# ishine/CatEars

Hardware: AMD Instinct MI355X
Metric: acoustic frames/sec (fbank->nnet posteriors), 16kHz, 1/2/4/8 GPU (higher is better)
Workload: dtype fp32 (bf16x6 GEMM: fp32 operands split exactly into 3 bf16 planes, 6 MFMA products, fp32 accumulate; every operand bit kept, dropped cross terms < 2^-25 |w x|; error vs oracle at the fp32-MFMA path's level, tests/test_gpu_parity.py)

## Files before the change

### catears_amd/csrc/kernels/gemm_bf16x6.hip

```cpp
#include <hip/hip_runtime.h>
#include <stdlib.h>

#include "../internal.h"
#include "../tile_order.h"

#ifndef CATEARS_X6_NT
#define CATEARS_X6_NT 0
#endif

namespace catears {
namespace {

typedef __bf16 bf16x8 __attribute__((ext_vector_type(8)));
typedef float f32x4 __attribute__((ext_vector_type(4)));
typedef float f32x2t __attribute__((ext_vector_type(2)));

struct X6Args {
  const uint16_t *w;
  const uint16_t *x;
  const float *wf, *xf;
  const float *bias, *bn_scale, *bn_offset;
  float *y32;
  uint16_t *y16;
  int ldw, pw, ldx, px, ldy, py;
// ... 420 lines not shown
          load_x(kt + 2, h);
          if (h == 1) read_plane(st, 2);
          __builtin_amdgcn_sched_barrier(0);
        }
#pragma unroll
        for (int i = 0; i < TW; ++i)
#pragma unroll
          for (int j = 0; j < TF; ++j) {
            acc[i][j] = __builtin_amdgcn_mfma_f32_16x16x32_bf16(a[0][i], b[2][j], acc[i][j], 0, 0, 0);
            acc[i][j] = __builtin_amdgcn_mfma_f32_16x16x32_bf16(a[2][i], b[0][j], acc[i][j], 0, 0, 0);
          }
        asm volatile("s_waitcnt lgkmcnt(0)" ::: "memory");
        __builtin_amdgcn_s_barrier();
      }
      asm volatile("s_waitcnt vmcnt(0)" ::: "memory");
      x6_epilogue<TW, TF, false>(p, acc, n0 + wrow, f0 + frow, lane);
      return;
    }
    for (int kt = 0; kt < ktiles; ++kt) {
      mfma_tile(kt);
      store(kt + 1);
      load(kt + 2);
      asm volatile("s_waitcnt lgkmcnt(0)" ::: "memory");
      if constexpr ((DIAG & 16) == 0) __builtin_amdgcn_s_barrier();
    }
    asm volatile("s_waitcnt vmcnt(0)" ::: "memory");
    x6_epilogue<TW, TF, false>(p, acc, n0 + wrow, f0 + frow, lane);
    return;
  }
  for (int kt = kbeg; kt < ktiles; ++kt) {
    store(kt + 1);
    load(kt + 2);
    const char *st = smem + (kt & 1) * STAGE;
    bf16x8 a[3][TW], b[3][TF];
#pragma unroll
    for (int pl = 0; pl < 3; ++pl) {
#pragma unroll
      for (int i = 0; i < TW; ++i)
        a[pl][i] = *reinterpret_cast<const bf16x8 *>(st + (pl * BW + wrow + i * 16) * 64 + foff);
#pragma unroll
      for (int j = 0; j < TF; ++j)
        b[pl][j] = *reinterpret_cast<const bf16x8 *>(st + 3 * BW * 64 + (pl * BF + frow + j * 16) * 64 + foff);
    }
#pragma unroll
    for (int i = 0; i < TW; ++i)
#pragma unroll
      for (int j = 0; j < TF; ++j) acc[i][j] = __builtin_amdgcn_mfma_f32_16x16x32_bf16(a[0][i], b[0][j], acc[i][j], 0, 0, 0);
#pragma unroll
    for (int i = 0; i < TW; ++i)
#pragma unroll
      for (int j = 0; j < TF; ++j) {
        acc[i][j] = __builtin_amdgcn_mfma_f32_16x16x32_bf16(a[0][i], b[1][j], acc[i][j], 0, 0, 0);
        acc[i][j] = __builtin_amdgcn_mfma_f32_16x16x32_bf16(a[1][i], b[0][j], acc[i][j], 0, 0, 0);
        acc[i][j] = __builtin_amdgcn_mfma_f32_16x16x32_bf16(a[1][i], b[1][j], acc[i][j], 0, 0, 0);
      }
#pragma unroll
    for (int i = 0; i < TW; ++i)
#pragma unroll
      for (int j = 0; j < TF; ++j) {
        acc[i][j] = __builtin_amdgcn_mfma_f32_16x16x32_bf16(a[0][i], b[2][j], acc[i][j], 0, 0, 0);
        acc[i][j] = __builtin_amdgcn_mfma_f32_16x16x32_bf16(a[2][i], b[0][j], acc[i][j], 0, 0, 0);
      }
    asm volatile("s_waitcnt lgkmcnt(0)" ::: "memory");
    __builtin_amdgcn_s_barrier();
  }
  asm volatile("s_waitcnt vmcnt(0)" ::: "memory");
  x6_epilogue<TW, TF, false>(p, acc, n0 + wrow, f0 + frow, lane);
}

template <class C, bool FIRST = false, int DIAG = 0, int KS = 1, bool PIN = false, bool OUT16 = false, int PRIO = 0>
__global__ __launch_bounds__(C::NT, 512 / C::NT) void gemm_bf16x6d_kernel(X6Args p) {
#ifndef CATEARS_DIAG
  static_assert(DIAG == 0, "ablation builds (wrong results) only with -DCATEARS_DIAG");
#endif
  static_assert(KS == 1 || (KS == 2 && !FIRST), "two K-tiles per stage: hidden layers only (even K-tile count)");
  static_assert(!PIN || (!FIRST && KS == 1 && DIAG == 0), "plane input: hidden / output layers, one K-tile per stage");
  constexpr int BF = C::BF, TW = C::TW, TF = C::TF, NT = C::NT;
  constexpr int RPP = NT / 4;
  static_assert(BF == RPP, "one activation row chunk per thread");
  constexpr int ASTAGE = 3 * BF * 64;
  __shared__ __attribute__((aligned(1024))) char smem[2 * KS * ASTAGE];
  auto stage_of = [&](int t) -> char * {
    if constexpr (KS == 1) return smem + (t & 1) * ASTAGE;
    else return smem + ((((t >> 1) & 1) << 1) + (t & 1)) * ASTAGE;
  };
  auto swz = [](int row) { return ((row >> 3) & 1) << 1; };
  typedef float f32x4v __attribute__((ext_vector_type(4)));
  typedef uint32_t u32x4 __attribute__((ext_vector_type(4)));
  typedef const __attribute__((address_space(1))) f32x4v gvec;
  typedef const __attribute__((address_space(1))) bf16x8 gfrag;
  typedef const __attribute__((address_space(1))) u32x4 gchunk;

  const int tid = threadIdx.x, lane = tid & 63, wave = tid >> 6;
  const int ww = wave / C::WGF, wf = wave % C::WGF;
  int tm, tn;
  tile_of(blockIdx.x, p.tiles_m, p.tiles_n, p.group, &tm, &tn);
  const int f0 = tm * BF, n0 = tn * C::BW;
  const int prow = tid >> 2, pch = tid & 3;
  const int ktiles = p.kpad / 32;

  gfrag *wb[TW];
#pragma unroll
  for (int i = 0; i < TW; ++i)
    wb[i] = (gfrag *)(p.wd + ((size_t)((n0 >> 4) + ww * TW + i) * p.wd_kt * 3 * 64 + lane) * 8);
  auto load_w = [&](int kt, int pl, bf16x8 *dst) {
    if constexpr ((DIAG & 8) != 0) {
      if (kt > 0) return;
    }
    kt = min(kt, ktiles - 1);
#pragma unroll
    for (int i = 0; i < TW; ++i) dst[i] = wb[i][(kt * 3 + pl) * 64];
  };
  f32x4v rx0[2], rx1[2];
  u32x4 rp[3][2];
  __shared__ int src_tab[FIRST ? 8 * BF : 1];
  if constexpr (FIRST) {
    for (int i = tid; i < 8 * BF; i += NT) {
      const int sg = i / BF, row = i % BF;
      const int shift = (int)(signed char)(p.off_packed >> (8 * min(sg, p.nseg - 1)));
      const int src = clampi(clampi(f0 + row, 0, p.m - 1) + shift, 0, p.m - 1);
      src_tab[i] = p.row_map ? p.row_map[src] : src;
    }
    __syncthreads();
  }
  auto load_x = [&](int kt, int r) {
    if constexpr ((DIAG & 4) != 0) {
      if (kt > 1) return;
    }
    kt = min(kt, ktiles - 1);
    const int k0 = kt * 32;
    if constexpr (FIRST) {
      const int k = k0 + 8 * pch, seg = k / p.din, segc = min(seg, p.nseg - 1);
      const int src = src_tab[segc * BF + prow];
      gvec *xb = (gvec *)(p.xf + (size_t)src * p.ldx + (seg < p.nseg ? k - segc * p.din : 0));
      rx0[r] = xb[0];
      rx1[r] = xb[1];
      if (seg >= p.nseg) rx0[r] = rx1[r] = f32x4v{0.0f, 0.0f, 0.0f, 0.0f};
    } else if constexpr (PIN) {
      const int seg = k0 / p.din, col0 = k0 - seg * p.din;
      const int shift = (int)(signed char)(p.off_packed >> (8 * seg));
      const int src = clampi(f0 + prow + shift, 0, p.m - 1);
      const uint32_t o = ((uint32_t)(src * p.ldx) + col0 + 8 * pch) / 8, ps = (uint32_t)p.px / 8;
      gchunk *xb = (gchunk *)p.x;
      rp[0][r] = xb[o];
      rp[1][r] = xb[o + ps];
      rp[2][r] = xb[o + 2 * ps];
    } else {
      const int seg = k0 / p.din, col0 = k0 - seg * p.din;
      const int shift = (int)(signed char)(p.off_packed >> (8 * seg));
      gvec *xb = (gvec *)(p.xf + col0 + 8 * pch);
      const int src = clampi(f0 + prow + shift, 0, p.m - 1);
      const uint32_t o = (uint32_t)(src * p.ldx) / 4;
      rx0[r] = xb[o];
      rx1[r] = xb[o + 1];
    }
  };
  auto put = [&](char *st, int r) {
    if constexpr ((DIAG & 2) != 0) return;
    if constexpr (PIN) {
      const int off = prow * 64 + ((pch ^ swz(prow)) * 16);
#pragma unroll
      for (int pl = 0; pl < 3; ++pl) *reinterpret_cast<u32x4 *>(st + pl * BF * 64 + off) = rp[pl][r];
      return;
    }
    Planes2 q0, q1, q2, q3;
    if constexpr ((DIAG & 1) != 0) {
      auto raw = [](float a, float b) {
        const uint32_t u = __builtin_bit_cast(uint32_t, a) ^ __builtin_bit_cast(uint32_t, b);
        return Planes2{u, u >> 1, u >> 2};
      };
      q0 = raw(rx0[r].x, rx0[r].y), q1 = raw(rx0[r].z, rx0[r].w);
      q2 = raw(rx1[r].x, rx1[r].y), q3 = raw(rx1[r].z, rx1[r].w);
    } else {
      q0 = split3_pair(rx0[r].x, rx0[r].y), q1 = split3_pair(rx0[r].z, rx0[r].w);
      q2 = split3_pair(rx1[r].x, rx1[r].y), q3 = split3_pair(rx1[r].z, rx1[r].w);
    }
    const int off = prow * 64 + ((pch ^ swz(prow)) * 16);
    *reinterpret_cast<u32x4 *>(st + off) = u32x4{q0.h, q1.h, q2.h, q3.h};
    *reinterpret_cast<u32x4 *>(st + BF * 64 + off) = u32x4{q0.m, q1.m, q2.m, q3.m};
    *reinterpret_cast<u32x4 *>(st + 2 * BF * 64 + off) = u32x4{q0.l, q1.l, q2.l, q3.l};
  };
  const int foff = (lane & 15) * 64 + (((lane >> 4) ^ (((lane >> 3) & 1) << 1)) * 16);
  const int frow = wf * TF * 16;
  auto read_b = [&](const char *st, int pl, bf16x8 *b) {
#pragma unroll
    for (int j = 0; j < TF; ++j) b[j] = *reinterpret_cast<const bf16x8 *>(st + (pl * BF + frow + j * 16) * 64 + foff);
  };

  f32x4 acc[TW][TF];
#pragma unroll
  for (int i = 0; i < TW; ++i)
#pragma unroll
    for (int j = 0; j < TF; ++j) acc[i][j] = f32x4{0.0f, 0.0f, 0.0f, 0.0f};

  bf16x8 a0[2][TW], a1[TW], a2[TW], b0[TF], b1[TF], b2[TF];
  load_x(0, 0);
  load_w(0, 0, a0[0]);
  load_w(0, 1, a1);
  load_w(0, 2, a2);
  if constexpr (KS == 1) {
    put(smem, 0);
    load_x(1, 1);
  } else {
    load_x(1, 1);
    put(stage_of(0), 0);
    put(stage_of(1), 1);
    load_x(2, 0);
  }
  asm volatile("s_waitcnt lgkmcnt(0)" ::: "memory");
  __builtin_amdgcn_s_barrier();

  auto body = [&](int kt, auto cc) {
    constexpr int c = decltype(cc)::value;
    const char *st = stage_of(kt);
    char *sn = stage_of(kt + KS);
    if constexpr (PRIO == 4) __builtin_amdgcn_s_setprio(1);
    read_b(st, 0, b0);
    read_b(st, 1, b1);
    if constexpr (PRIO == 4) __builtin_amdgcn_s_setprio(0);
    if constexpr (PRIO == 1 || PRIO == 3 || PRIO == 4 || PRIO == 5) __builtin_amdgcn_s_setprio(1);
    load_w(kt + 1, 0, a0[c ^ 1]);
    if constexpr (PRIO == 5) load_x(kt + KS + 1, KS == 1 ? c : c ^ 1);
    if constexpr (PRIO == 1 || PRIO == 3 || PRIO == 4 || PRIO == 5) __builtin_amdgcn_s_setprio(0);
    __builtin_amdgcn_sched_barrier(0);
    if constexpr (PRIO == 2) __builtin_amdgcn_s_setprio(1);
    if constexpr ((DIAG & 32) == 0) {
#pragma unroll
      for (int i = 0; i < TW; ++i)
#pragma unroll
        for (int j = 0; j < TF; ++j) acc[i][j] = __builtin_amdgcn_mfma_f32_16x16x32_bf16(a0[c][i], b0[j], acc[i][j], 0, 0, 0);
    }
    if constexpr (PRIO == 2) __builtin_amdgcn_s_setprio(0);
    __builtin_amdgcn_sched_barrier(0);
    if constexpr (PRIO == 1 || PRIO == 3 || PRIO == 4 || PRIO == 5) __builtin_amdgcn_s_setprio(1);
    if constexpr (PRIO != 5) load_x(kt + KS + 1, KS == 1 ? c : c ^ 1);
    if constexpr (PRIO == 1 || PRIO == 3 || PRIO == 4 || PRIO == 5) __builtin_amdgcn_s_setprio(0);
    __builtin_amdgcn_sched_barrier(0);
    if constexpr (PRIO == 2) __builtin_amdgcn_s_setprio(1);
    if constexpr (PRIO == 3) __builtin_amdgcn_s_setprio(1);
    put(sn, KS == 1 ? c ^ 1 : c);
    if constexpr (PRIO == 3) __builtin_amdgcn_s_setprio(0);
    if constexpr ((DIAG & 32) == 0) {
#pragma unroll
      for (int i = 0; i < TW; ++i)
#pragma unroll
        for (int j = 0; j < TF; ++j) {
          acc[i][j] = __builtin_amdgcn_mfma_f32_16x16x32_bf16(a0[c][i], b1[j], acc[i][j], 0, 0, 0);
          acc[i][j] = __builtin_amdgcn_mfma_f32_16x16x32_bf16(a1[i], b0[j], acc[i][j], 0, 0, 0);
          acc[i][j] = __builtin_amdgcn_mfma_f32_16x16x32_bf16(a1[i], b1[j], acc[i][j], 0, 0, 0);
        }
    }
    if constexpr (PRIO == 2) __builtin_amdgcn_s_setprio(0);
    if constexpr (PRIO == 4) __builtin_amdgcn_s_setprio(1);
    read_b(st, 2, b2);
    if constexpr (PRIO == 4) __builtin_amdgcn_s_setprio(0);
    __builtin_amdgcn_sched_barrier(0);
    if constexpr (PRIO == 1 || PRIO == 3 || PRIO == 4 || PRIO == 5) __builtin_amdgcn_s_setprio(1);
    load_w(kt + 1, 1, a1);
    if constexpr (PRIO == 1 || PRIO == 3 || PRIO == 4 || PRIO == 5) __builtin_amdgcn_s_setprio(0);
    __builtin_amdgcn_sched_barrier(0);
    if constexpr (PRIO == 2) __builtin_amdgcn_s_setprio(1);
    if constexpr ((DIAG & 32) == 0) {
#pragma unroll
      for (int i = 0; i < TW; ++i)
#pragma unroll
        for (int j = 0; j < TF; ++j) {
          acc[i][j] = __builtin_amdgcn_mfma_f32_16x16x32_bf16(a0[c][i], b2[j], acc[i][j], 0, 0, 0);
          acc[i][j] = __builtin_amdgcn_mfma_f32_16x16x32_bf16(a2[i], b0[j], acc[i][j], 0, 0, 0);
        }
    } else {
#pragma unroll
      for (int j = 0; j < TF; ++j) acc[0][j][0] += (float)b0[j][0] + (float)b1[j][0] + (float)b2[j][0] +
                                                   (float)a0[c][0][0] + (float)a1[0][0] + (float)a2[0][0];
    }
    if constexpr (PRIO == 2) __builtin_amdgcn_s_setprio(0);
    __builtin_amdgcn_sched_barrier(0);
    if constexpr (PRIO == 1 || PRIO == 3 || PRIO == 4 || PRIO == 5) __builtin_amdgcn_s_setprio(1);
    load_w(kt + 1, 2, a2);
    if constexpr (PRIO == 1 || PRIO == 3 || PRIO == 4 || PRIO == 5) __builtin_amdgcn_s_setprio(0);
    if constexpr (KS == 1 || c == 1) {
      asm volatile("s_waitcnt lgkmcnt(0)" ::: "memory");
      if constexpr ((DIAG & 16) == 0) __builtin_amdgcn_s_barrier();
    }
    __builtin_amdgcn_sched_barrier(0);
  };
  int kt = 0;
  for (; kt + 1 < ktiles; kt += 2) {
    body(kt, std::integral_constant<int, 0>());
    body(kt + 1, std::integral_constant<int, 1>());
  }
  if (KS == 1 && kt < ktiles) body(kt, std::integral_constant<int, 0>());
  asm volatile("s_waitcnt vmcnt(0)" ::: "memory");
  x6_epilogue<TW, TF, OUT16>(p, acc, n0 + ww * TW * 16, f0 + frow, lane);
}

template <int BW_, int BF_, int WGW_, int WGF_>
struct W6Cfg {
  static constexpr int BW = BW_, BF = BF_, WGW = WGW_, WGF = WGF_;
  static constexpr int NW = WGW * WGF, NT = 64 * NW;
  static constexpr int TW = BW / WGW / 16, TF = BF / WGF / 16;
  static_assert(TW * WGW * 16 == BW && TF * WGF * 16 == BF, "bad one-wave-per-SIMD tile");
};

template <class C, bool SG = false, int RING = 4>
__global__ __launch_bounds__(C::NT, C::NW / 4) void gemm_bf16x6w_kernel(X6Args p) {
  constexpr int BF = C::BF, TW = C::TW, TF = C::TF, NT = C::NT;
  static_assert(C::NW == 4 || C::NW == 8, "one or two waves per SIMD");
  static_assert(TW % RING == 0, "a ring of unit-block weight buffers that divides the unit blocks");
  constexpr int RQ = BF / (NT / 4);
  static_assert(RQ >= 1 && RQ * (NT / 4) == BF, "whole activation rows per thread");
  constexpr int ASTAGE = 3 * BF * 64;
  __shared__ __attribute__((aligned(1024))) char smem[2 * ASTAGE];
  auto swz = [](int row) { return ((row >> 3) & 1) << 1; };
  typedef float f32x4v __attribute__((ext_vector_type(4)));
  typedef uint32_t u32x4 __attribute__((ext_vector_type(4)));
  typedef const __attribute__((address_space(1))) f32x4v gvec;
  typedef const __attribute__((address_space(1))) bf16x8 gfrag;

  const int tid = threadIdx.x, lane = tid & 63, wave = tid >> 6;
  const int ww = wave / C::WGF, wf = wave % C::WGF;
  int tm, tn;
  tile_of(blockIdx.x, p.tiles_m, p.tiles_n, p.group, &tm, &tn);
  const int f0 = tm * BF, n0 = tn * C::BW;
  const int prow = tid >> 2, pch = tid & 3;
  const int ktiles = p.kpad / 32;

  gfrag *wbase = (gfrag *)(p.wd + ((size_t)((n0 >> 4) + ww * TW) * p.wd_kt * 3 * 64 + lane) * 8);
  bf16x8 wa[RING][3];
  auto load_w = [&](int kt, int i, int buf) {
    kt = min(kt, ktiles - 1);
#pragma unroll
    for (int pl = 0; pl < 3; ++pl) wa[buf][pl] = wbase[((size_t)(i * p.wd_kt + kt) * 3 + pl) * 64];
  };
  f32x4v rx0[RQ], rx1[RQ];
  auto load_x = [&](int kt) {
    kt = min(kt, ktiles - 1);
    const int k0 = kt * 32;
    const int seg = k0 / p.din, col0 = k0 - seg * p.din;
    const int shift = (int)(signed char)(p.off_packed >> (8 * seg));
    gvec *xb = (gvec *)(p.xf + col0 + 8 * pch);
#pragma unroll
    for (int q = 0; q < RQ; ++q) {
      const int src = clampi(f0 + prow + q * (NT / 4) + shift, 0, p.m - 1);
      const uint32_t o = (uint32_t)(src * p.ldx) / 4;
      rx0[q] = xb[o];
      rx1[q] = xb[o + 1];
    }
  };
  auto put = [&](char *st) {
#pragma unroll
    for (int q = 0; q < RQ; ++q) {
      const Planes2 q0 = split3_pair(rx0[q].x, rx0[q].y), q1 = split3_pair(rx0[q].z, rx0[q].w);
      const Planes2 q2 = split3_pair(rx1[q].x, rx1[q].y), q3 = split3_pair(rx1[q].z, rx1[q].w);
      const int row = prow + q * (NT / 4);
      const int off = row * 64 + ((pch ^ swz(row)) * 16);
      *reinterpret_cast<u32x4 *>(st + off) = u32x4{q0.h, q1.h, q2.h, q3.h};
      *reinterpret_cast<u32x4 *>(st + BF * 64 + off) = u32x4{q0.m, q1.m, q2.m, q3.m};
      *reinterpret_cast<u32x4 *>(st + 2 * BF * 64 + off) = u32x4{q0.l, q1.l, q2.l, q3.l};
    }
  };
  const int foff = (lane & 15) * 64 + (((lane >> 4) ^ (((lane >> 3) & 1) << 1)) * 16);
  const int frow = wf * TF * 16;
  auto frag = [&](const char *st, int pl, int j) {
    return *reinterpret_cast<const bf16x8 *>(st + (pl * BF + frow + j * 16) * 64 + foff);
  };

  f32x4 acc[TW][TF];
#pragma unroll
  for (int i = 0; i < TW; ++i)
#pragma unroll
    for (int j = 0; j < TF; ++j) acc[i][j] = f32x4{0.0f, 0.0f, 0.0f, 0.0f};
  bf16x8 b0[TF], b1[TF], b2[TF];

  load_x(0);
#pragma unroll
  for (int i = 0; i < RING - 1; ++i) load_w(0, i, i);
  put(smem);
  load_x(1);
  asm volatile("s_waitcnt lgkmcnt(0)" ::: "memory");
  __builtin_amdgcn_s_barrier();
#pragma unroll
  for (int j = 0; j < TF; ++j) {
    b0[j] = frag(smem, 0, j);
    b1[j] = frag(smem, 1, j);
    b2[j] = frag(smem, 2, j);
  }

  for (int kt = 0; kt < ktiles; ++kt) {
    char *sn = smem + ((kt + 1) & 1) * ASTAGE;
#pragma unroll
    for (int i = 0; i < TW; ++i) {
      load_w(kt + (i + RING - 1) / TW, (i + RING - 1) % TW, (i + RING - 1) % RING);
      if (i == 0) {
        if constexpr (!SG) {
          put(sn);
          load_x(kt + 2);
        }
      }
      __builtin_amdgcn_sched_barrier(0);
      if constexpr (SG) {
        if (i == 0) {
          put(sn);
          load_x(kt + 2);
#pragma unroll
          for (int g = 0; g < 6 * TF; ++g) {
            __builtin_amdgcn_sched_group_barrier(0x008, 1, 0);
            __builtin_amdgcn_sched_group_barrier(0x002, 2, 0);
            if (g % 4 == 3) __builtin_amdgcn_sched_group_barrier(0x200, 1, 0);
          }
        }
      }
      constexpr int u = 0;
#pragma unroll
      for (int j = 0; j < TF; ++j) {
        acc[i][j] = __builtin_amdgcn_mfma_f32_16x16x32_bf16(wa[i % RING][u], b0[j], acc[i][j], 0, 0, 0);
        acc[i][j] = __builtin_amdgcn_mfma_f32_16x16x32_bf16(wa[i % RING][u], b1[j], acc[i][j], 0, 0, 0);
        acc[i][j] = __builtin_amdgcn_mfma_f32_16x16x32_bf16(wa[i % RING][u + 1], b0[j], acc[i][j], 0, 0, 0);
        acc[i][j] = __builtin_amdgcn_mfma_f32_16x16x32_bf16(wa[i % RING][u + 1], b1[j], acc[i][j], 0, 0, 0);
        acc[i][j] = __builtin_amdgcn_mfma_f32_16x16x32_bf16(wa[i % RING][u], b2[j], acc[i][j], 0, 0, 0);
        acc[i][j] = __builtin_amdgcn_mfma_f32_16x16x32_bf16(wa[i % RING][u + 2], b0[j], acc[i][j], 0, 0, 0);
        if (i == TW - 1) {
          b0[j] = frag(sn, 0, j);
          b1[j] = frag(sn, 1, j);
          b2[j] = frag(sn, 2, j);
        }
      }
      if constexpr (SG) {
        if (i == TW - 1) {
#pragma unroll
          for (int j = 0; j < TF; ++j) {
            __builtin_amdgcn_sched_group_barrier(0x008, 6, 0);
            __builtin_amdgcn_sched_group_barrier(0x100, 3, 0);
          }
        }
      }
      if (i == TW / 2 - 1) {
        asm volatile("s_waitcnt lgkmcnt(0)" ::: "memory");
        __builtin_amdgcn_s_barrier();
      }
      __builtin_amdgcn_sched_barrier(0);
    }
  }
  asm volatile("s_waitcnt vmcnt(0) lgkmcnt(0)" ::: "memory");
  x6_epilogue<TW, TF, false>(p, acc, n0 + ww * TW * 16, f0 + frow, lane);
}

#ifdef CATEARS_EXPERIMENTS
template <class C>
__global__ __launch_bounds__(C::NT, 1) void gemm_bf16x6r_kernel(X6Args p) {
  constexpr int TW = C::TW, TF = C::TF;
  typedef float f32x4v __attribute__((ext_vector_type(4)));
  typedef uint32_t u32x4 __attribute__((ext_vector_type(4)));
  typedef const __attribute__((address_space(1))) f32x4v gvec;
  typedef const __attribute__((address_space(1))) bf16x8 gfrag;
  const int lane = threadIdx.x & 63, wave = threadIdx.x >> 6;
  const int ww = wave / C::WGF, wf = wave % C::WGF;
  int tm, tn;
  tile_of(blockIdx.x, p.tiles_m, p.tiles_n, p.group, &tm, &tn);
  const int f0 = tm * C::BF + wf * TF * 16, n0 = tn * C::BW;
  const int ktiles = p.kpad / 32;
  gfrag *wb[TW];
#pragma unroll
  for (int i = 0; i < TW; ++i)
    wb[i] = (gfrag *)(p.wd + ((size_t)((n0 >> 4) + ww * TW + i) * p.wd_kt * 3 * 64 + lane) * 8);
  int xrow[TF];
#pragma unroll
  for (int j = 0; j < TF; ++j) xrow[j] = f0 + 16 * j + (lane & 15);
  bf16x8 a[2][3][TW];
  f32x4v x[2][TF][2];
  auto load = [&](int kt, int buf) {
    kt = min(kt, ktiles - 1);
#pragma unroll
    for (int pl = 0; pl < 3; ++pl)
#pragma unroll
      for (int i = 0; i < TW; ++i) a[buf][pl][i] = wb[i][(kt * 3 + pl) * 64];
    const int k0 = kt * 32;
    const int seg = k0 / p.din, col = k0 - seg * p.din + 8 * (lane >> 4);
    const int shift = (int)(signed char)(p.off_packed >> (8 * seg));
#pragma unroll
    for (int j = 0; j < TF; ++j) {
      const int src = clampi(xrow[j] + shift, 0, p.m - 1);
      gvec *xp = (gvec *)(p.xf + (size_t)src * p.ldx + col);
      x[buf][j][0] = xp[0];
      x[buf][j][1] = xp[1];
    }
  };
  f32x4 acc[TW][TF];
#pragma unroll
  for (int i = 0; i < TW; ++i)
#pragma unroll
    for (int j = 0; j < TF; ++j) acc[i][j] = f32x4{0.0f, 0.0f, 0.0f, 0.0f};
  auto compute = [&](int buf) {
#pragma unroll
    for (int j = 0; j < TF; ++j) {
      const f32x4v v0 = x[buf][j][0], v1 = x[buf][j][1];
      const Planes2 q0 = split3_pair(v0.x, v0.y), q1 = split3_pair(v0.z, v0.w);
      const Planes2 q2 = split3_pair(v1.x, v1.y), q3 = split3_pair(v1.z, v1.w);
      const bf16x8 b0 = __builtin_bit_cast(bf16x8, u32x4{q0.h, q1.h, q2.h, q3.h});
      const bf16x8 b1 = __builtin_bit_cast(bf16x8, u32x4{q0.m, q1.m, q2.m, q3.m});
      const bf16x8 b2 = __builtin_bit_cast(bf16x8, u32x4{q0.l, q1.l, q2.l, q3.l});
#pragma unroll
      for (int i = 0; i < TW; ++i) acc[i][j] = __builtin_amdgcn_mfma_f32_16x16x32_bf16(a[buf][0][i], b0, acc[i][j], 0, 0, 0);
#pragma unroll
      for (int i = 0; i < TW; ++i) acc[i][j] = __builtin_amdgcn_mfma_f32_16x16x32_bf16(a[buf][0][i], b1, acc[i][j], 0, 0, 0);
#pragma unroll
      for (int i = 0; i < TW; ++i) acc[i][j] = __builtin_amdgcn_mfma_f32_16x16x32_bf16(a[buf][1][i], b0, acc[i][j], 0, 0, 0);
#pragma unroll
      for (int i = 0; i < TW; ++i) acc[i][j] = __builtin_amdgcn_mfma_f32_16x16x32_bf16(a[buf][1][i], b1, acc[i][j], 0, 0, 0);
#pragma unroll
      for (int i = 0; i < TW; ++i) acc[i][j] = __builtin_amdgcn_mfma_f32_16x16x32_bf16(a[buf][0][i], b2, acc[i][j], 0, 0, 0);
#pragma unroll
      for (int i = 0; i < TW; ++i) acc[i][j] = __builtin_amdgcn_mfma_f32_16x16x32_bf16(a[buf][2][i], b0, acc[i][j], 0, 0, 0);
    }
  };
  load(0, 0);
  int kt = 0;
  for (; kt + 1 < ktiles; kt += 2) {
    load(kt + 1, 1);
    __builtin_amdgcn_sched_barrier(0);
    compute(0);
    __builtin_amdgcn_sched_barrier(0);
    load(kt + 2, 0);
    __builtin_amdgcn_sched_barrier(0);
    compute(1);
    __builtin_amdgcn_sched_barrier(0);
  }
  if (kt < ktiles) compute(0);
  asm volatile("s_waitcnt vmcnt(0)" ::: "memory");
  x6_epilogue<TW, TF, false>(p, acc, n0 + ww * TW * 16, f0, lane);
}

#endif

template <class C, int NPV>
__global__ __launch_bounds__(C::NT + 64 * NPV, 1) void gemm_bf16x6ws_kernel(X6Args p) {
  constexpr int BW = C::BW, BF = C::BF, TW = C::TW, TF = C::TF, NT = C::NT, STAGE = C::STAGE;
  constexpr int RPP = 16 * NPV;
  static_assert((BW + BF) % RPP == 0, "rows per pass");
  constexpr int NP = (BW + BF) / RPP;
  __shared__ __attribute__((aligned(1024))) char smem[2 * STAGE];
  auto swz = [](int row) { return ((row >> 3) & 1) << 1; };
  typedef float f32x4v __attribute__((ext_vector_type(4)));
  typedef uint32_t u32x4 __attribute__((ext_vector_type(4)));
  typedef const __attribute__((address_space(1))) f32x4v gvec;

  const int tid = threadIdx.x, lane = tid & 63;
  const int wave = __builtin_amdgcn_readfirstlane(tid >> 6);
  int tm, tn;
  tile_of(blockIdx.x, p.tiles_m, p.tiles_n, p.group, &tm, &tn);
  const int f0 = tm * BF, n0 = tn * BW;
  const int ktiles = p.kpad / 32;

  if (wave >= C::NW) {
    const int pt = tid - NT, prow = pt >> 2, pch = pt & 3;
    bool isw[NP];
    int trow[NP];
    uint32_t wsrc[NP];
    int dst[NP];
#pragma unroll
    for (int i = 0; i < NP; ++i) {
      const int r = i * RPP + prow;
      isw[i] = BW % RPP == 0 ? i < BW / RPP : r < BW;
      trow[i] = isw[i] ? r : r - BW;
      wsrc[i] = (uint32_t)(min(n0 + trow[i], p.n - 1) * p.ldw + 8 * pch);
      dst[i] = (isw[i] ? 0 : 3 * BW * 64) + trow[i] * 64 + ((pch ^ swz(trow[i])) * 16);
    }
    f32x4v r0[NP], r1[NP];
    auto load = [&](int kt) {
      kt = min(kt, ktiles - 1);
      const int k0 = kt * 32;
      const int seg = k0 / p.din, col0 = k0 - seg * p.din;
      const int shift = (int)(signed char)(p.off_packed >> (8 * seg));
#pragma unroll
      for (int i = 0; i < NP; ++i) {
        gvec *src;
        if (isw[i]) {
          src = (gvec *)(p.wf + k0 + wsrc[i]);
        } else {
          const int x = clampi(f0 + trow[i] + shift, 0, p.m - 1);
          src = (gvec *)(p.xf + (uint32_t)(x * p.ldx) + col0 + 8 * pch);
        }
        r0[i] = src[0];
        r1[i] = src[1];
      }
    };
    auto store = [&](int kt) {
      char *st = smem + (kt & 1) * STAGE;
#pragma unroll
      for (int i = 0; i < NP; ++i) {
        const f32x4v v0 = r0[i], v1 = r1[i];
        const Planes2 q0 = split3_pair(v0.x, v0.y), q1 = split3_pair(v0.z, v0.w);
        const Planes2 q2 = split3_pair(v1.x, v1.y), q3 = split3_pair(v1.z, v1.w);
        const int ps = (isw[i] ? BW : BF) * 64;
        char *d = st + dst[i];
        *reinterpret_cast<u32x4 *>(d) = u32x4{q0.h, q1.h, q2.h, q3.h};
        *reinterpret_cast<u32x4 *>(d + ps) = u32x4{q0.m, q1.m, q2.m, q3.m};
        *reinterpret_cast<u32x4 *>(d + 2 * ps) = u32x4{q0.l, q1.l, q2.l, q3.l};
      }
    };
    load(0);
    store(0);
    load(1);
    asm volatile("s_waitcnt lgkmcnt(0)" ::: "memory");
    __builtin_amdgcn_s_barrier();
    for (int kt = 0; kt < ktiles; ++kt) {
      store(kt + 1);
      load(kt + 2);
      asm volatile("s_waitcnt lgkmcnt(0)" ::: "memory");
      __builtin_amdgcn_s_barrier();
    }
    asm volatile("s_waitcnt vmcnt(0)" ::: "memory");
    return;
  }

  const int ww = wave / C::WGF, wf = wave % C::WGF;
  const int foff = (lane & 15) * 64 + (((lane >> 4) ^ (((lane >> 3) & 1) << 1)) * 16);
  const int wrow = ww * TW * 16, frow = wf * TF * 16;
  f32x4 acc[TW][TF];
#pragma unroll
  for (int i = 0; i < TW; ++i)
#pragma unroll
    for (int j = 0; j < TF; ++j) acc[i][j] = f32x4{0.0f, 0.0f, 0.0f, 0.0f};
  __builtin_amdgcn_s_barrier();
  for (int kt = 0; kt < ktiles; ++kt) {
    const char *st = smem + (kt & 1) * STAGE;
    bf16x8 a[3][TW], b[3][TF];
#pragma unroll
    for (int pl = 0; pl < 3; ++pl) {
#pragma unroll
      for (int i = 0; i < TW; ++i)
        a[pl][i] = *reinterpret_cast<const bf16x8 *>(st + (pl * BW + wrow + i * 16) * 64 + foff);
#pragma unroll
      for (int j = 0; j < TF; ++j)
        b[pl][j] = *reinterpret_cast<const bf16x8 *>(st + 3 * BW * 64 + (pl * BF + frow + j * 16) * 64 + foff);
    }
#pragma unroll
    for (int i = 0; i < TW; ++i)
#pragma unroll
      for (int j = 0; j < TF; ++j) acc[i][j] = __builtin_amdgcn_mfma_f32_16x16x32_bf16(a[0][i], b[0][j], acc[i][j], 0, 0, 0);
#pragma unroll
    for (int i = 0; i < TW; ++i)
#pragma unroll
      for (int j = 0; j < TF; ++j) {
        acc[i][j] = __builtin_amdgcn_mfma_f32_16x16x32_bf16(a[0][i], b[1][j], acc[i][j], 0, 0, 0);
        acc[i][j] = __builtin_amdgcn_mfma_f32_16x16x32_bf16(a[1][i], b[0][j], acc[i][j], 0, 0, 0);
        acc[i][j] = __builtin_amdgcn_mfma_f32_16x16x32_bf16(a[1][i], b[1][j], acc[i][j], 0, 0, 0);
      }
#pragma unroll
    for (int i = 0; i < TW; ++i)
#pragma unroll
      for (int j = 0; j < TF; ++j) {
        acc[i][j] = __builtin_amdgcn_mfma_f32_16x16x32_bf16(a[0][i], b[2][j], acc[i][j], 0, 0, 0);
        acc[i][j] = __builtin_amdgcn_mfma_f32_16x16x32_bf16(a[2][i], b[0][j], acc[i][j], 0, 0, 0);
      }
    asm volatile("s_waitcnt lgkmcnt(0)" ::: "memory");
    __builtin_amdgcn_s_barrier();
  }
  x6_epilogue<TW, TF, false>(p, acc, n0 + wrow, f0 + frow, lane);
}

struct SpliceIdx8 {
  int v[8];
};

__global__ __launch_bounds__(256) void splice_pad_split_kernel(const float *__restrict__ in, int ld_in, int rows,
                                                               int din, int nseg, SpliceIdx8 idx,
                                                               const int *__restrict__ row_map,
                                                               uint16_t *__restrict__ out, int po) {
  const int r = blockIdx.x * 4 + (threadIdx.x >> 6), lane = threadIdx.x & 63;
  if (r >= rows) return;
  uint16_t *o = out + (int64_t)r * 3 * po;
  for (int c = lane; c < po; c += 64) {
    const int s = c / din;
    float v = 0.0f;
    if (s < nseg) {
      int src = clampi(r + idx.v[s], 0, rows - 1);
      if (row_map) src = row_map[src];
      v = in[(int64_t)src * ld_in + (c - s * din)];
    }
    uint16_t h, m, l;
    split3(v, &h, &m, &l);
    o[c] = h;
    o[po + c] = m;
    o[2 * po + c] = l;
  }
}

template <class C, int SCHED>
int launch_q(hipStream_t s, X6Args p, bool out16) {
  p.tiles_n = (p.n + C::BW - 1) / C::BW;
  p.tiles_m = (p.m + C::BF - 1) / C::BF;
  dim3 grid(p.tiles_m * p.tiles_n), block(C::NT);
  if (out16)
    hipLaunchKernelGGL((gemm_bf16x6q_kernel<C, true, SCHED>), grid, block, 0, s, p);
  else
    hipLaunchKernelGGL((gemm_bf16x6q_kernel<C, false, SCHED>), grid, block, 0, s, p);
  CE_HIP(hipGetLastError());
  return CE_GPU_OK;
}

template <class C, int SCHED = 0, int DIAG = 0>
int launch_f(hipStream_t s, X6Args p) {
  p.tiles_n = (p.n + C::BW - 1) / C::BW;
  p.tiles_m = (p.m + C::BF - 1) / C::BF;
  dim3 grid(p.tiles_m * p.tiles_n), block(C::NT);
  hipLaunchKernelGGL((gemm_bf16x6f_kernel<C, SCHED, DIAG>), grid, block, 0, s, p);
  CE_HIP(hipGetLastError());
  return CE_GPU_OK;
}

#ifdef CATEARS_EXPERIMENTS
template <class C>
int launch_r(hipStream_t s, X6Args p) {
  p.tiles_n = (p.n + C::BW - 1) / C::BW;
  p.tiles_m = (p.m + C::BF - 1) / C::BF;
  dim3 grid(p.tiles_m * p.tiles_n), block(C::NT);
  hipLaunchKernelGGL((gemm_bf16x6r_kernel<C>), grid, block, 0, s, p);
  CE_HIP(hipGetLastError());
  return CE_GPU_OK;
}
#endif

int x6_ks() {
  static int v = CE_KNOB("CATEARS_X6_KS", 1);
  return v;
}

template <class C, int DIAG = 0, int PRIO = 0>
int launch_d(hipStream_t s, X6Args p) {
  p.tiles_n = (p.n + C::BW - 1) / C::BW;
  p.tiles_m = (p.m + C::BF - 1) / C::BF;
  dim3 grid(p.tiles_m * p.tiles_n), block(C::NT);
  const bool out16 = p.y16 != nullptr;
  if (p.row_map || p.din % 32 != 0) {
    if (out16)
      hipLaunchKernelGGL((gemm_bf16x6d_kernel<C, true, 0, 1, false, true>), grid, block, 0, s, p);
    else
      hipLaunchKernelGGL((gemm_bf16x6d_kernel<C, true>), grid, block, 0, s, p);
  } else if (!p.xf) {
    if (out16)
      hipLaunchKernelGGL((gemm_bf16x6d_kernel<C, false, 0, 1, true, true>), grid, block, 0, s, p);
    else
      hipLaunchKernelGGL((gemm_bf16x6d_kernel<C, false, 0, 1, true, false>), grid, block, 0, s, p);
  } else if (out16) {
    hipLaunchKernelGGL((gemm_bf16x6d_kernel<C, false, 0, 1, false, true>), grid, block, 0, s, p);
  } else if (x6_ks() == 2 && (p.kpad / 32) % 2 == 0)
    hipLaunchKernelGGL((gemm_bf16x6d_kernel<C, false, DIAG, 2>), grid, block, 0, s, p);
  else
    hipLaunchKernelGGL((gemm_bf16x6d_kernel<C, false, DIAG, 1, false, false, PRIO>), grid, block, 0, s, p);
  CE_HIP(hipGetLastError());
  return CE_GPU_OK;
}

constexpr int kX6WideMinTiles = 48;

int x6w_group(int tiles_n) {
  static int v = CE_KNOB("CATEARS_X6W_GROUP", 0);
  return v > 0 ? v : (tiles_n <= 2 ? 1 : 2);
}

template <class C, bool SG = false, int RING = 4>
bool launch_w(hipStream_t s, X6Args p, int min_tiles = 0) {
  p.tiles_n = (p.n + C::BW - 1) / C::BW;
  p.tiles_m = (p.m + C::BF - 1) / C::BF;
  if ((p.n + 255) / 256 * 256 < p.tiles_n * C::BW) return false;
  if (p.tiles_n * p.tiles_m < min_tiles) return false;
  p.group = x6w_group(p.tiles_n);
  hipLaunchKernelGGL((gemm_bf16x6w_kernel<C, SG, RING>), dim3(p.tiles_m * p.tiles_n), dim3(C::NT), 0, s, p);
  return true;
}

template <class C, int NPV>
int launch_ws(hipStream_t s, X6Args p) {
  p.tiles_n = (p.n + C::BW - 1) / C::BW;
  p.tiles_m = (p.m + C::BF - 1) / C::BF;
  dim3 grid(p.tiles_m * p.tiles_n), block(C::NT + 64 * NPV);
  hipLaunchKernelGGL((gemm_bf16x6ws_kernel<C, NPV>), grid, block, 0, s, p);
  CE_HIP(hipGetLastError());
  return CE_GPU_OK;
}

int x6_variant() {
  static int v = CE_KNOB("CATEARS_X6_VARIANT", 0);
  return v;
}

int x6_first_tile() {
  static int v = CE_KNOB("CATEARS_X6_FIRST_TILE", 128);
  return v;
}

}

int launch_gemm_bf16x6(hipStream_t s, const X6Gemm &a) {
  if (a.m <= 0 || a.n <= 0) return CE_GPU_OK;
  const bool first = a.row_map != nullptr || a.din % 32 != 0;
  if (a.kpad % 32 != 0 || a.din % (first ? 8 : 32) != 0 || a.din <= 0 || a.nseg < 1 || a.nseg > 8 ||
      a.nseg * a.din > a.kpad)
    return fail(CE_GPU_EINVAL, "gemm_bf16x6: bad K geometry");
  if (first && (!a.xf || !a.wd || (x6_variant() != 0 && x6_variant() != 300 && (x6_variant() < 310 || x6_variant() > 316))))
    return fail(CE_GPU_EINVAL, "gemm_bf16x6: a gathered first layer needs fp32 input and the direct-weight kernel");
  if (a.n % 4 != 0 || a.ldy % 4 != 0 || (a.y16 && a.py % 4 != 0))
    return fail(CE_GPU_EINVAL, "gemm_bf16x6: output width must be a multiple of 4");
  const bool f32in = a.xf != nullptr;
  const bool direct = a.wd && (x6_variant() == 0 || x6_variant() == 300);
  const bool pin = !f32in && a.x && a.wd;
  if (pin) {
    if (!direct || first || a.ldx % 8 || a.px % 8 || (reinterpret_cast<uintptr_t>(a.x) & 15) ||
        (int64_t)a.m * a.ldx >= ((int64_t)1 << 31) || (int64_t)a.m * a.ldy >= ((int64_t)1 << 31))
      return fail(CE_GPU_EINVAL, "gemm_bf16x6: plane input needs the direct-weight kernel, din % 32 == 0, "
                                 "16-byte aligned planes and 2^31-element operands");
  }
  if (a.y16 && f32in && !direct)
    return fail(CE_GPU_EINVAL, "gemm_bf16x6: fp32 input with split output needs the direct-weight kernel");
  if (f32in) {
    if (!a.wf || !(a.y32 || a.y16) || a.ldw % 4 || a.ldx % 4 || (reinterpret_cast<uintptr_t>(a.wf) & 15) ||
        (reinterpret_cast<uintptr_t>(a.xf) & 15))
      return fail(CE_GPU_EINVAL, "gemm_bf16x6: fp32 operands must be 16-byte aligned, output fp32");
    if ((int64_t)a.n * a.ldw >= ((int64_t)1 << 31) || (int64_t)a.m * a.ldx >= ((int64_t)1 << 31) ||
        (int64_t)a.m * a.ldy >= ((int64_t)1 << 31))
      return fail(CE_GPU_EINVAL, "gemm_bf16x6: operand beyond 2^31 elements");
  } else {
    if (a.ldw % 8 || a.pw % 8 || a.ldx % 8 || a.px % 8 || (reinterpret_cast<uintptr_t>(a.w) & 15) ||
        (reinterpret_cast<uintptr_t>(a.x) & 15))
      return fail(CE_GPU_EINVAL, "gemm_bf16x6: operands must be 16-byte aligned");
    if ((int64_t)a.n * a.ldw * 2 >= ((int64_t)1 << 32) || (int64_t)a.m * a.ldx * 2 >= ((int64_t)1 << 32))
      return fail(CE_GPU_EINVAL, "gemm_bf16x6: operand beyond 4 GiB");
  }
  if (a.npost > 4) return fail(CE_GPU_EINVAL, "gemm_bf16x6: too many post ops");
  X6Args p;
  p.w = a.w;
  p.x = a.x;
  p.wf = a.wf;
  p.xf = a.xf;
  p.bias = a.bias;
  p.bn_scale = a.bn_scale;
  p.bn_offset = a.bn_offset;
  p.y32 = a.y32;
  p.y16 = a.y16;
  p.ldw = a.ldw;
  p.pw = a.pw;
  p.ldx = a.ldx;
  p.px = a.px;
  p.ldy = a.ldy;
  p.py = a.py;
  p.m = a.m;
  p.n = a.n;
  p.kpad = a.kpad;
  p.din = a.din;
  p.nseg = a.nseg;
  p.row_map = a.row_map;
  p.off_packed = 0;
  for (int i = 0; i < a.nseg; ++i) {
    if (a.off[i] < -128 || a.off[i] > 127) return fail(CE_GPU_ENOTSUP, "gemm_bf16x6: splice offset beyond +-127");
    p.off_packed |= (uint64_t)(uint8_t)(int8_t)a.off[i] << (8 * i);
  }
  for (int i = 0; i < 4; ++i) p.post[i] = a.post[i];
  p.npost = a.npost;
  p.post_mode = post_mode(a.post, a.npost);
#ifndef CATEARS_X6_GROUP
#define CATEARS_X6_GROUP 2
#endif
  p.group = CATEARS_X6_GROUP;
  p.wd = a.wd;
  p.wd_kt = a.wd_kt;
  const bool out16 = a.y16 != nullptr;
  if (pin || (f32in && out16)) {
    if (a.wd_kt * 32 < a.kpad || (reinterpret_cast<uintptr_t>(a.wd) & 15))
      return fail(CE_GPU_EINVAL, "gemm_bf16x6: weight fragment image does not cover K");
    if (a.wide || (first && x6_first_tile() == 128)) return launch_d<X6Cfg<128, 128, 2, 4, 2>>(s, p);
    return launch_d<X6Cfg<kX6DirUnits, 128, 4, 2, 2>>(s, p);
  }
  if (f32in) {
    switch (x6_variant()) {
      case 0:
      case 300:
        if (a.wd) {
          if (a.wd_kt * 32 < a.kpad || (reinterpret_cast<uintptr_t>(a.wd) & 15))
            return fail(CE_GPU_EINVAL, "gemm_bf16x6: weight fragment image does not cover K");
          if (a.wide || (first && x6_first_tile() == 128)) return launch_d<X6Cfg<128, 128, 2, 4, 2>>(s, p);
          if (x6_variant() == 0 && !first && launch_w<W6Cfg<512, 128, 4, 2>, true>(s, p, kX6WideMinTiles)) {
            CE_HIP(hipGetLastError());
            return CE_GPU_OK;
          }
          return launch_d<X6Cfg<kX6DirUnits, 128, 4, 2, 2>>(s, p);
        }
        [[fallthrough]];
      case 160:
        return launch_f<X6Cfg<128, 256, 2, 4, 2>, 8>(s, p);
#ifdef CATEARS_EXPERIMENTS
      case 40:
        return launch_f<X6Cfg<128, 128, 4, 2, 2>>(s, p);
      case 200:
        return launch_ws<X6Cfg<128, 128, 2, 2, 2>, 4>(s, p);
      case 400:
        if (!a.wd || a.wd_kt * 32 < a.kpad || (reinterpret_cast<uintptr_t>(a.wd) & 15))
          return fail(CE_GPU_EINVAL, "variant 400 needs the weight fragment image");
        return launch_r<X6Cfg<kX6DirUnits, 128, 4, 2, 2>>(s, p);
      case 302:
        if (!a.wd) return fail(CE_GPU_EINVAL, "variant 302 needs the weight fragment image");
        return launch_d<X6Cfg<128, 128, 2, 4, 2>>(s, p);
      case 320:
        if (!a.wd) return fail(CE_GPU_EINVAL, "variant 320 needs the weight fragment image");
        if (first) return launch_d<X6Cfg<128, 128, 2, 4, 2>>(s, p);
        return launch_d<X6Cfg<kX6DirUnits, 128, 8, 1, 2>>(s, p);
      case 340:
        if (!a.wd) return fail(CE_GPU_EINVAL, "variant 340 needs the weight fragment image");
        if (first) return launch_d<X6Cfg<128, 128, 2, 4, 2>>(s, p);
        return launch_d<X6Cfg<kX6DirUnits, 64, 4, 1, 2>>(s, p);
      case 331:
      case 332:
      case 333:
      case 334:
      case 335:
        if (!a.wd) return fail(CE_GPU_EINVAL, "variants 331-335 need the weight fragment image");
        if (first) return launch_d<X6Cfg<128, 128, 2, 4, 2>>(s, p);
        if (x6_variant() == 331) return launch_d<X6Cfg<kX6DirUnits, 128, 4, 2, 2>, 0, 1>(s, p);
        if (x6_variant() == 333) return launch_d<X6Cfg<kX6DirUnits, 128, 4, 2, 2>, 0, 3>(s, p);
        if (x6_variant() == 334) return launch_d<X6Cfg<kX6DirUnits, 128, 4, 2, 2>, 0, 4>(s, p);
        if (x6_variant() == 335) return launch_d<X6Cfg<kX6DirUnits, 128, 4, 2, 2>, 0, 5>(s, p);
        return launch_d<X6Cfg<kX6DirUnits, 128, 4, 2, 2>, 0, 2>(s, p);
#endif
#if defined(CATEARS_EXPERIMENTS) || defined(CATEARS_X6W)
      case 500:
      case 501:
      case 502:
      case 503:
      case 504:
      case 505:
      case 506:
      case 507:
      case 508: {
        if (!a.wd || a.wd_kt * 32 < a.kpad) return fail(CE_GPU_EINVAL, "variants 500-503 need the weight fragment image");
        if (first || a.wide) return launch_d<X6Cfg<128, 128, 2, 4, 2>>(s, p);
        const int v = x6_variant();
        const bool ok = v == 500   ? launch_w<W6Cfg<512, 128, 4, 1>>(s, p)
                        : v == 504 ? launch_w<W6Cfg<512, 128, 4, 1>, true>(s, p)
                        : v == 505 ? launch_w<W6Cfg<512, 64, 4, 1>, true>(s, p)
                        : v == 506 ? launch_w<W6Cfg<512, 64, 4, 1>, true, 8>(s, p)
                        : v == 507 ? launch_w<W6Cfg<256, 128, 4, 1>, true>(s, p)
                        : v == 508 ? launch_w<W6Cfg<512, 128, 4, 2>, true>(s, p)
                        : v == 501 ? launch_w<W6Cfg<512, 64, 4, 1>>(s, p)
                        : v == 502 ? launch_w<W6Cfg<256, 128, 4, 1>>(s, p)
                                   : launch_w<W6Cfg<256, 256, 2, 2>>(s, p);
        if (!ok) return launch_d<X6Cfg<kX6DirUnits, 128, 4, 2, 2>>(s, p);
        CE_HIP(hipGetLastError());
        return CE_GPU_OK;
      }
#endif
#ifdef CATEARS_EXPERIMENTS
      case 42:
        return launch_f<X6Cfg<128, 256, 2, 4, 2>>(s, p);
      case 55:
        return launch_f<X6Cfg<128, 256, 2, 4, 2>, 6>(s, p);
      case 202:
        return launch_ws<X6Cfg<128, 256, 2, 2, 2>, 4>(s, p);
      case 204:
        return launch_ws<X6Cfg<128, 256, 2, 4, 2>, 4>(s, p);
#endif
#ifdef CATEARS_DIAG
      case 310:
      case 311:
      case 312:
      case 313:
      case 314:
      case 315:
      case 316: {
        if (!a.wd) return fail(CE_GPU_EINVAL, "ablations of 300 need the weight fragment image");
        using D = X6Cfg<kX6DirUnits, 128, 4, 2, 2>;
        if (first) return launch_d<X6Cfg<128, 128, 2, 4, 2>>(s, p);
        switch (x6_variant()) {
          case 310: return launch_d<D, 1>(s, p);
          case 311: return launch_d<D, 2>(s, p);
          case 312: return launch_d<D, 6>(s, p);
          case 313: return launch_d<D, 8>(s, p);
          case 314: return launch_d<D, 16>(s, p);
          case 315: return launch_d<D, 32>(s, p);
          default: return launch_d<D, 2 | 4 | 8 | 16>(s, p);
        }
      }
      case 91:
        return launch_f<X6Cfg<128, 256, 2, 4, 2>, 6, 1>(s, p);
      case 92:
        return launch_f<X6Cfg<128, 256, 2, 4, 2>, 6, 2>(s, p);
      case 94:
        return launch_f<X6Cfg<128, 256, 2, 4, 2>, 6, 4>(s, p);
      case 96:
        return launch_f<X6Cfg<128, 256, 2, 4, 2>, 6, 16>(s, p);
      case 98:
        return launch_f<X6Cfg<128, 256, 2, 4, 2>, 6, 8>(s, p);
      case 99:
        return launch_f<X6Cfg<128, 256, 2, 4, 2>, 6, 3>(s, p);
      case 100:
        return launch_f<X6Cfg<128, 256, 2, 4, 2>, 6, 27>(s, p);
      case 101:
        return launch_f<X6Cfg<128, 256, 2, 4, 2>, 6, 59>(s, p);
      case 102:
        return launch_f<X6Cfg<128, 256, 2, 4, 2>, 6, 32>(s, p);
      case 103:
        return launch_f<X6Cfg<128, 256, 2, 4, 2>, 6, 43>(s, p);
#endif
      default:
        return fail(CE_GPU_EINVAL, "bf16x6 schedule " + std::to_string(x6_variant()) +
                                       " is not in this build (the experiments library: `make EXPERIMENTS=1`)");
    }
  }
  return launch_q<X6Cfg<128, 128, 4, 2, 3>, 0>(s, p, out16);
}

int launch_splice_pad_split(hipStream_t s, const float *in, int ld_in, int rows, int din, int nseg, const int *off,
                            const int *row_map, uint16_t *out, int po) {
  if (nseg < 1 || nseg > 8 || nseg * din > po) return fail(CE_GPU_EINVAL, "splice_pad_split: bad geometry");
  SpliceIdx8 idx = {};
  for (int i = 0; i < nseg; ++i) idx.v[i] = off[i];
  if (rows > 0)
    hipLaunchKernelGGL(splice_pad_split_kernel, dim3((rows + 3) / 4), dim3(256), 0, s, in, ld_in, rows, din, nseg,
                       idx, row_map, out, po);
  CE_HIP(hipGetLastError());
  return CE_GPU_OK;
}

}
```

Baseline: 7.008 million.

## Add peeled wide bf16x6 k-loop with scalar weight addressing and placed LDS writes

Adds a PEEL variant of the wide bf16x6 kernel, enabled on the default launch path. The per-k-tile body is rewritten with explicit sched_group_barrier interleaving of MFMAs, LDS reads and LDS writes at fixed slots. The wave index becomes scalar via readfirstlane, and the weight fragment address is built from a scalar base plus a 32-bit lane offset to cut 64-bit vector address arithmetic. Precomputed LDS store offsets are pinned in VGPRs. The hand-placed schedule depends on exact tile sizes (static_assert) and may interact with register pressure or hazards.

```diff
diff --git a/catears_amd/csrc/kernels/gemm_bf16x6.hip b/catears_amd/csrc/kernels/gemm_bf16x6.hip
--- a/catears_amd/csrc/kernels/gemm_bf16x6.hip
+++ b/catears_amd/csrc/kernels/gemm_bf16x6.hip
@@ -746,10 +746,11 @@
   static_assert(TW * WGW * 16 == BW && TF * WGF * 16 == BF, "bad one-wave-per-SIMD tile");
 };
 
-template <class C, bool SG = false, int RING = 4>
+template <class C, bool SG = false, int RING = 4, bool PEEL = false>
 __global__ __launch_bounds__(C::NT, C::NW / 4) void gemm_bf16x6w_kernel(X6Args p) {
   constexpr int BF = C::BF, TW = C::TW, TF = C::TF, NT = C::NT;
   static_assert(C::NW == 4 || C::NW == 8, "one or two waves per SIMD");
+  static_assert(!PEEL || (SG && TF == 4 && BF == NT / 4), "the peeled loop's write slots are placed for 24 MFMAs and one row chunk");
   static_assert(TW % RING == 0, "a ring of unit-block weight buffers that divides the unit blocks");
   constexpr int RQ = BF / (NT / 4);
   static_assert(RQ >= 1 && RQ * (NT / 4) == BF, "whole activation rows per thread");
@@ -761,7 +762,8 @@
   typedef const __attribute__((address_space(1))) f32x4v gvec;
   typedef const __attribute__((address_space(1))) bf16x8 gfrag;
 
-  const int tid = threadIdx.x, lane = tid & 63, wave = tid >> 6;
+  const int tid = threadIdx.x, lane = tid & 63;
+  const int wave = PEEL ? __builtin_amdgcn_readfirstlane(tid >> 6) : tid >> 6;
   const int ww = wave / C::WGF, wf = wave % C::WGF;
   int tm, tn;
   tile_of(blockIdx.x, p.tiles_m, p.tiles_n, p.group, &tm, &tn);
@@ -770,11 +772,19 @@
   const int ktiles = p.kpad / 32;
 
   gfrag *wbase = (gfrag *)(p.wd + ((size_t)((n0 >> 4) + ww * TW) * p.wd_kt * 3 * 64 + lane) * 8);
+  const __attribute__((address_space(1))) char *wscalar =
+      (const __attribute__((address_space(1))) char *)p.wd + (size_t)((n0 >> 4) + ww * TW) * p.wd_kt * 3 * 1024;
+  const uint32_t wlane = lane * 16;
   bf16x8 wa[RING][3];
   auto load_w = [&](int kt, int i, int buf) {
     kt = min(kt, ktiles - 1);
 #pragma unroll
-    for (int pl = 0; pl < 3; ++pl) wa[buf][pl] = wbase[((size_t)(i * p.wd_kt + kt) * 3 + pl) * 64];
+    for (int pl = 0; pl < 3; ++pl) {
+      if constexpr (PEEL)
+        wa[buf][pl] = ((gfrag *)(wscalar + (uint32_t)((i * p.wd_kt + kt) * 3072) + wlane))[pl * 64];
+      else
+        wa[buf][pl] = wbase[((size_t)(i * p.wd_kt + kt) * 3 + pl) * 64];
+    }
   };
   f32x4v rx0[RQ], rx1[RQ];
   auto load_x = [&](int kt) {
@@ -790,6 +800,17 @@
       rx0[q] = xb[o];
       rx1[q] = xb[o + 1];
     }
+  };
+  auto put_off = [&](int q) {
+    const int row = prow + q * (NT / 4);
+    return row * 64 + ((pch ^ swz(row)) * 16);
+  };
+  auto put_to = [&](char *d, int q) {
+    const Planes2 q0 = split3_pair(rx0[q].x, rx0[q].y), q1 = split3_pair(rx0[q].z, rx0[q].w);
+    const Planes2 q2 = split3_pair(rx1[q].x, rx1[q].y), q3 = split3_pair(rx1[q].z, rx1[q].w);
+    *reinterpret_cast<u32x4 *>(d) = u32x4{q0.h, q1.h, q2.h, q3.h};
+    *reinterpret_cast<u32x4 *>(d + BF * 64) = u32x4{q0.m, q1.m, q2.m, q3.m};
+    *reinterpret_cast<u32x4 *>(d + 2 * BF * 64) = u32x4{q0.l, q1.l, q2.l, q3.l};
   };
   auto put = [&](char *st) {
 #pragma unroll
@@ -828,6 +849,67 @@
     b0[j] = frag(smem, 0, j);
     b1[j] = frag(smem, 1, j);
     b2[j] = frag(smem, 2, j);
+  }
+
+  if constexpr (PEEL) {
+    auto ktile = [&](int kt) __attribute__((always_inline)) {
+      char *sn = smem + ((kt + 1) & 1) * ASTAGE;
+      uint32_t pdst[RQ];
+#pragma unroll
+      for (int i = 0; i < TW; ++i) {
+        load_w(kt + (i + RING - 1) / TW, (i + RING - 1) % TW, (i + RING - 1) % RING);
+        if (i == 0) {
+#pragma unroll
+          for (int q = 0; q < RQ; ++q) {
+            pdst[q] = (uint32_t)(((kt + 1) & 1) * ASTAGE + put_off(q));
+            asm volatile("" : "+v"(pdst[q]));
+          }
+        }
+        __builtin_amdgcn_sched_barrier(0);
+        if (i == 0) {
+#pragma unroll
+          for (int q = 0; q < RQ; ++q) put_to(smem + pdst[q], q);
+          load_x(kt + 2);
+#pragma unroll
+          for (int g = 0; g < 6 * TF; ++g) {
+            __builtin_amdgcn_sched_group_barrier(0x008, 1, 0);
+            __builtin_amdgcn_sched_group_barrier(0x002, 2, 0);
+            if (g == 18 || g == 21 || g == 23) __builtin_amdgcn_sched_group_barrier(0x200, 1, 0);
+          }
+        }
+#pragma unroll
+        for (int j = 0; j < TF; ++j) {
+          acc[i][j] = __builtin_amdgcn_mfma_f32_16x16x32_bf16(wa[i % RING][0], b0[j], acc[i][j], 0, 0, 0);
+          acc[i][j] = __builtin_amdgcn_mfma_f32_16x16x32_bf16(wa[i % RING][0], b1[j], acc[i][j], 0, 0, 0);
+          acc[i][j] = __builtin_amdgcn_mfma_f32_16x16x32_bf16(wa[i % RING][1], b0[j], acc[i][j], 0, 0, 0);
+          acc[i][j] = __builtin_amdgcn_mfma_f32_16x16x32_bf16(wa[i % RING][1], b1[j], acc[i][j], 0, 0, 0);
+          acc[i][j] = __builtin_amdgcn_mfma_f32_16x16x32_bf16(wa[i % RING][0], b2[j], acc[i][j], 0, 0, 0);
+          acc[i][j] = __builtin_amdgcn_mfma_f32_16x16x32_bf16(wa[i % RING][2], b0[j], acc[i][j], 0, 0, 0);
+          if (i == TW - 1) {
+            b0[j] = frag(sn, 0, j);
+            b1[j] = frag(sn, 1, j);
+            b2[j] = frag(sn, 2, j);
+          }
+        }
+        if (i == TW - 1) {
+#pragma unroll
+          for (int j = 0; j < TF; ++j) {
+            __builtin_amdgcn_sched_group_barrier(0x008, 6, 0);
+            __builtin_amdgcn_sched_group_barrier(0x100, 3, 0);
+          }
+        }
+        if (i == TW / 2 - 1) {
+          asm volatile("s_waitcnt lgkmcnt(0)" ::: "memory");
+          __builtin_amdgcn_s_barrier();
+        }
+        __builtin_amdgcn_sched_barrier(0);
+      }
+    };
+    ktile(0);
+    for (int kt = 1; kt < ktiles; ++kt) ktile(kt);
+    asm volatile("s_waitcnt vmcnt(0) lgkmcnt(0)" ::: "memory");
+    x6_epilogue<TW, TF, false>(p, acc, n0 + ww * TW * 16, f0 + frow, lane);
+    return;
   }
 
   for (int kt = 0; kt < ktiles; ++kt) {
@@ -1203,14 +1285,14 @@
   return v > 0 ? v : (tiles_n <= 2 ? 1 : 2);
 }
 
-template <class C, bool SG = false, int RING = 4>
+template <class C, bool SG = false, int RING = 4, bool PEEL = false>
 bool launch_w(hipStream_t s, X6Args p, int min_tiles = 0) {
   p.tiles_n = (p.n + C::BW - 1) / C::BW;
   p.tiles_m = (p.m + C::BF - 1) / C::BF;
   if ((p.n + 255) / 256 * 256 < p.tiles_n * C::BW) return false;
   if (p.tiles_n * p.tiles_m < min_tiles) return false;
   p.group = x6w_group(p.tiles_n);
-  hipLaunchKernelGGL((gemm_bf16x6w_kernel<C, SG, RING>), dim3(p.tiles_m * p.tiles_n), dim3(C::NT), 0, s, p);
+  hipLaunchKernelGGL((gemm_bf16x6w_kernel<C, SG, RING, PEEL>), dim3(p.tiles_m * p.tiles_n), dim3(C::NT), 0, s, p);
   return true;
 }
 
@@ -1323,7 +1405,7 @@
           if (a.wd_kt * 32 < a.kpad || (reinterpret_cast<uintptr_t>(a.wd) & 15))
             return fail(CE_GPU_EINVAL, "gemm_bf16x6: weight fragment image does not cover K");
           if (a.wide || (first && x6_first_tile() == 128)) return launch_d<X6Cfg<128, 128, 2, 4, 2>>(s, p);
-          if (x6_variant() == 0 && !first && launch_w<W6Cfg<512, 128, 4, 2>, true>(s, p, kX6WideMinTiles)) {
+          if (x6_variant() == 0 && !first && launch_w<W6Cfg<512, 128, 4, 2>, true, 4, true>(s, p, kX6WideMinTiles)) {
             CE_HIP(hipGetLastError());
             return CE_GPU_OK;
           }
```

Result: no change. 7.008 million, median of 4 (-0.0%).
